# ksadov/FREUD

Measured on AMD Instinct MI355X. Metric: SAE train activations/sec (d=384 dict 8x), higher is better.
Workload: dtype bf16; 1 GPU; Whisper-tiny d=384 dict 8x (n=3072) L1 SAE train step, M=65536 rows/GPU/step, RAdam+cosine, x bfloat16 resident in HBM (BASELINE configs[1]); rows_per_gpu=65536, d_model=384, n_dict=3072, parallelism=dp1, dp=none

## Files before the change

freud_amd/csrc/engine.hip:

```cpp
#include <hip/hip_runtime.h>
#include <math.h>
#include <stdarg.h>
#include <stdio.h>
#include <string.h>

#include <algorithm>
#include <utility>
#include <vector>

#include "../../include/freud_sae.h"
#include "l1_kernels.h"
#include "gemm256.h"
#include "gemm256s.h"
#include "gemm256_fp8.h"
#include "l1_fp8.h"
#include "dp_kernels.h"
#include "p2p_exchange.h"
#include <rccl/rccl.h>
#include <mutex>
#include <unistd.h>

static thread_local bool g_force_gemm128 = false;
static thread_local bool g_no_stream = false;
static thread_local int g_device = 0;
// ... 49 lines not shown
  do {                                                                        \
    int rc_ = ensure_lds_attr(reinterpret_cast<const void*>(fn), (bytes), (device)); \
    if (rc_) return rc_;                                                      \
  } while (0)

static int grid_for(int64_t n, int cap, int per = 256) {
  const int64_t g = (n + per - 1) / per;
  return (int)(g < cap ? g : cap);
}

template <class F>
static int with_x_type(int x_dtype, const void* x, F&& f) {
  switch (x_dtype) {
    case SAE_DTYPE_F32: return f((const float*)x);
    case SAE_DTYPE_F16: return f((const _Float16*)x);
    case SAE_DTYPE_BF16: return f((const bf16_t*)x);
    default: return fail(SAE_ERR_INVALID, "unknown x_dtype %d", x_dtype);
  }
}

enum KernelId {
  KID_PREP_W = 0,
  KID_PREP_X,
  KID_ENC_FWD,
  KID_DEC_FWD,
  KID_FWD_FUSED,
  KID_DPRE,
  KID_DW,
  KID_BWD_FUSED,
  KID_REDUCE,
  KID_OPT,
  KID_TK_ENC,
  KID_TK_SELECT,
  KID_TK_DECODE,
  KID_TK_DDENSE,
  KID_TK_DWD,
  KID_TK_DWE,
  KID_TK_DSAE,
  KID_TK_AUX,
  KID_EXCHANGE,
  KID_STATS_XCHG,
  KID_STEP_TOTAL,
  KID_COACT_PACK,
  KID_COACT_UPDATE,
  KID_MANIP_SERIES,
  KID_MANIP_DECODE,
  KID_MANIP_APPLY,
  KID_LABEL_PACK,
  KID_LABEL_UPDATE,
  KID_COUNT
};
static const char* kKernelNames[KID_COUNT] = {"prep_w", "prep_x", "enc_fwd_gemm", "dec_fwd_gemm", "fwd_fused_gemm", "dpre_gemm",
                                              "dw_gemm", "bwd_fused_gemm", "reduce_grads", "clip_adam", "topk_enc_gemm", "topk_select",
                                              "topk_decode", "topk_ddense_gemm", "topk_dwdec_gemm", "topk_dwenc_gemm",
                                              "topk_dsaein_colsum", "topk_auxk_backward", "dp_exchange", "dp_stats_exchange",
                                              "fwd_bwd_total", "coact_pack", "coact_update", "manip_series", "manip_decode",
                                              "manip_apply", "label_pack", "label_update"};
constexpr int EV_RING = 64;

struct EvRing {
  hipEvent_t beg[EV_RING], end[EV_RING];
  int n = 0;
};

enum LastCall { LAST_FWD_BF16 = 0, LAST_FWD_E32, LAST_SEARCH, LAST_STATS, LAST_COACT, LAST_LABELS };

struct sae_ctx {
  sae_config cfg;
  int d, n, d_p, n_p;
  int64_t max_rows_p;
  int64_t nW;
  int64_t nparams;
  float *P = nullptr, *Mom = nullptr, *Var = nullptr;
  float* G = nullptr;
  bf16_t *Wb = nullptr, *Wt = nullptr;
  bool fp8 = false;
  bool fp8_bwd = false;
  unsigned char* dxh8 = nullptr;
  int row_pad = 128;
  unsigned char *x8 = nullptr, *c8 = nullptr, *W8 = nullptr, *W8t = nullptr;
  float *scal8 = nullptr, *x8_part = nullptr;
  bool use_fused_fwd = false;
  int fwd_variant = 2;
  bf16_t *xb = nullptr, *c = nullptr, *dxh = nullptr, *dpre = nullptr;
  bf16_t *dxhT = nullptr, *xT = nullptr;
  float *slab = nullptr, *db_part = nullptr, *l1_part = nullptr, *sq_part = nullptr, *scal = nullptr;
  double* gn_part = nullptr;
  float* cn_part = nullptr;
  bool cn_valid = false;
  bool wb_valid = false;
  float* cnorm = nullptr;
  bool wn_pending = false, wn_fwd_seen = false;
  sae_grad_ready_fn grad_ready = nullptr;
  void* grad_ready_user = nullptr;
  int dw_chunk_rows = 0;
  int dw_chunk_splits = 1;
  int dw_col_chunks = 1;
  int dw_col_splits = 1;
  float* cnt_part = nullptr;
  int gn_blocks = 0;
  bool step_fused_call = false;
  bool gn_valid = false;
  bool metrics_fresh = false;
  const bf16_t* xb_cur = nullptr;
  unsigned int* masked = nullptr;
  int dw_splits = 1;
  int dw_tail_tiles = 0, dw_tail_pieces = 0;
  float* dw_tail = nullptr;
  int bwd_splits = 1;
  int bwd_range_splits = 1;
  bool use_fused_bwd = false;
  bool topk = false;
  int k = 0, k_aux_cap = 0;
  int64_t rows_per_file = 0;
  double dead_threshold = 1e300;
  bf16_t *We_b = nullptr, *Wd_b = nullptr, *xs = nullptr, *pre = nullptr, *dense = nullptr, *aux_dense = nullptr;
  bf16_t *de_b = nullptr, *dh_b = nullptr;
  float *e = nullptr, *dh = nullptr, *e2_part = nullptr, *a2_part = nullptr, *dbd_part = nullptr, *ds_part = nullptr, *tkf = nullptr;
  int *top_idx = nullptr, *aux_idx = nullptr, *tk = nullptr;
  bf16_t *top_vals = nullptr, *aux_vals = nullptr, *multi_vals = nullptr;
  unsigned short* tile_max = nullptr;
  unsigned char* sel_flag = nullptr;
  bool dense_valid = false;
  bool multi_dense_valid = false;
  float* be_r = nullptr;
  int slab_splits = 1;
  bool aux_compact = false;
  int *tkd = nullptr, *dead_cols = nullptr, *vec_rank = nullptr;
  unsigned char* vec_bits = nullptr;
  bf16_t* Wdd_b = nullptr;
  float* aux_dbe_part = nullptr;
  int* dead_hint = nullptr;
  double* tv_part = nullptr;
  long long* nfsf = nullptr;
  long long* dbe_fx = nullptr;
  bool topk_sparse_da = false;
  bool topk_csc = false;
  unsigned short* csc_counts = nullptr;
  unsigned int *csc_block_off = nullptr, *csc_total = nullptr, *csc_start = nullptr, *csc_item_start = nullptr, *csc_item_latent = nullptr;
  unsigned int* csc_multi = nullptr;
  CscEntry* csc_entries = nullptr;
  float *csc_part = nullptr, *csc_pbe = nullptr;
  int64_t csc_max_items = 0;
  bool multi = false;
  int k4 = 0;
  bf16_t *multi_dense = nullptr, *dm_b = nullptr;
  int* multi_idx = nullptr;
  float *em = nullptr, *m2_part = nullptr;
  unsigned char* dead = nullptr;
  double* stats = nullptr;
  int64_t stats_cap = 0, stats_n = 0;
  unsigned int* stats_part = nullptr;
  int dp_world = 0;
  bool dist = false;
  ncclComm_t comm = nullptr;
  hipStream_t comm_stream = nullptr;
  hipEvent_t ev_x = nullptr, ev_stats = nullptr, ev_done = nullptr;
  hipEvent_t ev_range[16] = {};
  int ev_range_i = 0;
  int payload = SAE_DTYPE_F32;
  bf16_t* Gb = nullptr;
  bool grads_in_bf16 = false;
  int dist_error = 0;
  char dist_errmsg[256] = "";
  bool p2p = false;
  int p2p_rank = 0;
// ... 296 lines not shown
        if (r.beg[i]) (void)hipEventDestroy(r.beg[i]);
        if (r.end[i]) (void)hipEventDestroy(r.end[i]);
      }
  delete c;
}

extern "C" int sae_create(const sae_config* cfg, sae_ctx** out) {
  if (!cfg || !out) return fail(SAE_ERR_INVALID, "null argument");
  *out = nullptr;
  if (cfg->variant != SAE_VARIANT_L1 && cfg->variant != SAE_VARIANT_TOPK)
    return fail(SAE_ERR_INVALID, "Invalid autoencoder variant: %d, must be 'l1' or 'topk'", cfg->variant);
  if (cfg->variant == SAE_VARIANT_TOPK && (cfg->k <= 0 || cfg->k > cfg->n_dict || cfg->k > 1024))
    return fail(SAE_ERR_INVALID, "topk: k=%d must be in [1, min(n_dict, 1024)]", cfg->k);
  if (cfg->variant == SAE_VARIANT_TOPK && cfg->multi_topk && (4 * cfg->k > cfg->n_dict || 4 * cfg->k > 1024))
    return fail(SAE_ERR_INVALID, "topk: multi_topk selects 4k = %d latents, must be <= min(n_dict, 1024)", 4 * cfg->k);
  if (cfg->variant != SAE_VARIANT_TOPK && cfg->multi_topk)
    return fail(SAE_ERR_INVALID, "multi_topk is a TopK option");
  if (cfg->variant == SAE_VARIANT_TOPK && cfg->d_model > 1536)
    return fail(SAE_ERR_INVALID, "topk: d_model=%d above the 1536 the sparse decoder is built for", cfg->d_model);
  if (cfg->d_model <= 0 || cfg->n_dict <= 0 || cfg->max_rows <= 0)
    return fail(SAE_ERR_INVALID, "d_model, n_dict and max_rows must be positive");
  if (cfg->optimizer != SAE_OPT_RADAM && cfg->optimizer != SAE_OPT_ADAM)
    return fail(SAE_ERR_INVALID, "Invalid optimizer: %d, must be 'radam' or 'adam'", cfg->optimizer);
  int ndev = 0;
  HIP_TRY(hipGetDeviceCount(&ndev));
  if (cfg->device_id < 0 || cfg->device_id >= ndev) return fail(SAE_ERR_INVALID, "device_id %d out of range", cfg->device_id);
  HIP_TRY(hipSetDevice(cfg->device_id));
  g_device = cfg->device_id;

  if (cfg->precision != SAE_PREC_BF16 && cfg->precision != SAE_PREC_FP8 && cfg->precision != SAE_PREC_FP8_BWD)
    return fail(SAE_ERR_INVALID, "Invalid precision: %d, must be SAE_PREC_BF16, SAE_PREC_FP8 or SAE_PREC_FP8_BWD", cfg->precision);
  if (cfg->precision != SAE_PREC_BF16 && cfg->variant != SAE_VARIANT_L1)
    return fail(SAE_ERR_INVALID, "fp8 encoder / decoder GEMMs exist for the L1 variant only");

  sae_ctx* c = new sae_ctx();
  c->cfg = *cfg;
  c->d = cfg->d_model;
  c->n = cfg->n_dict;
  c->fp8 = cfg->precision != SAE_PREC_BF16;
  c->fp8_bwd = cfg->precision == SAE_PREC_FP8_BWD;
  const int pad = c->fp8 ? 256 : 128;
  c->row_pad = pad;
  c->d_p = (int)round_up(c->d, pad);
  c->n_p = (int)round_up(c->n, pad);
  c->max_rows_p = round_up(cfg->max_rows, pad);
  c->nW = (int64_t)c->d_p * c->n_p;
  c->nparams = c->nW + c->n_p;
  c->topk = cfg->variant == SAE_VARIANT_TOPK;
  if (const char* fg = getenv("FREUD_P2P_FINEGRAINED")) c->finegrained = atoi(fg) == 1;
  const int64_t Mp = c->max_rows_p;
  if (c->topk) {
    int rc_tk = topk_create(c, Mp);
    if (rc_tk) {
      sae_destroy(c);
      return rc_tk;
    }
    *out = c;
    return SAE_OK;
  }
  g_force_gemm128 = cfg->force_gemm128 == 1;
  c->no_stream = g_no_stream = cfg->debug_flags == 86 || (getenv("FREUD_GEMM_STREAM") && atoi(getenv("FREUD_GEMM_STREAM")) == 0);
  c->dw_splits = choose_splits(c->d_p / 128, c->n_p / 128, 2 * Mp / 64);
  if (const char* ov = getenv("FREUD_DW_SPLITS")) {
    const int v = atoi(ov);
    if (v >= 1 && v <= 64) c->dw_splits = v;
  }
  c->dw_chunk_rows = c->d_p >= 1024 ? 512 : c->d_p;
  if (!g_force_gemm128 && c->d_p % 256 == 0 && c->n_p % 256 == 0 && (c->d_p / 256) * (c->n_p / 256) >= 256 && !getenv("FREUD_DW_SPLITS") &&
      c->cfg.debug_flags != 81) {
    gemm_tail_plan((c->d_p / 256) * (c->n_p / 256), (int)(2 * Mp / 64), c->dw_tail_tiles, c->dw_tail_pieces);
    if ((c->d_p / 256) * (c->n_p / 256) % 256 == 0) c->dw_tail_tiles = c->dw_tail_pieces = -1;
  }
  c->dw_chunk_splits = choose_splits(c->dw_chunk_rows / 128, c->n_p / 128, 2 * Mp / 64);
  if (c->d_p >= 1024 && c->n_p % 256 == 0)
    for (int q = 4; q >= 2; --q)
      if ((c->n_p / 256) % q == 0) {
        c->dw_col_chunks = q;
        break;
      }
  c->dw_col_splits = choose_splits(c->d_p / 128, c->n_p / 128 / c->dw_col_chunks, 2 * Mp / 64);
  c->use_fused_bwd = (c->d_p == BF_D) && cfg->force_generic != 1 && !c->fp8;
  c->use_fused_fwd = (c->d_p == FF_D) && cfg->force_generic != 1 && !c->fp8;
  if (const char* fv = getenv("FREUD_FWD")) c->fwd_variant = atoi(fv) == 1 ? 1 : 2;
  c->bwd_splits = fused_bwd_splits(c->n_p / BF_BN, (int)(Mp / BF_BM), c->n_p);
  c->bwd_range_splits = c->bwd_splits;
  for (int r = 2; r <= 4; ++r)
    if ((c->n_p / BF_BN) % r == 0) {
      const int sp = fused_bwd_splits(c->n_p / BF_BN / r, (int)(Mp / BF_BM), c->n_p / r);
      if (sp > c->bwd_range_splits) c->bwd_range_splits = sp;
    }
  int slab_splits = c->use_fused_bwd ? (c->bwd_range_splits > c->dw_splits ? c->bwd_range_splits : c->dw_splits) : c->dw_splits;
  if (c->use_fused_bwd && c->cfg.debug_flags != 83 && !getenv("FREUD_BWD_UNIFORM")) {
    const int ntiles = c->n_p / BF_BN, cus = 256;
    const int m = (32 * ntiles + cus - 1) / cus, grid = (32 * ntiles + m - 1) / m;
    int pmax = 1;
    for (int j = 0; j < ntiles; ++j) pmax = bal_pieces(j, m) > pmax ? bal_pieces(j, m) : pmax;
    const int steps = (int)(Mp / BF_BM), q = (steps + 31) / 32;
    const double slab_steps = (double)c->n_p * BF_D * 8.0 / 4.0e12 / 1.43e-6;
    const double cost_bal = (double)m * q + 5.0 + (32 % m ? 3.5 : 0.0) + (32.0 / m + (32 % m ? 1.0 : 0.0)) * slab_steps;
    const int sp = c->bwd_splits, rounds = (ntiles * sp + 255) / 256;
    const double cost_uni = rounds * ((double)((steps + sp - 1) / sp) + 5.0) + sp * slab_steps;
    if (cost_bal < cost_uni * 0.995 && pmax <= 64 && grid <= 4096) {
      c->bal_m = m;
      c->bal_grid = grid;
      if (pmax > slab_splits) slab_splits = pmax;
      std::vector<int> order(grid);
      for (int k = 0; k < grid; ++k) order[k] = k;
      std::stable_sort(order.begin(), order.end(), [m](int a_, int b_) { return (a_ * m) % 32 < (b_ * m) % 32; });
      std::vector<short> map(grid);
      int pos = 0;
      for (int x = 0; x < 8; ++x) {
        const int len = grid / 8 + (x < grid % 8 ? 1 : 0);
        for (int i = 0; i < len; ++i) map[8 * i + x] = (short)order[pos++];
      }
      hipError_t e_ = hipMalloc((void**)&c->bal_map, (size_t)grid * 2);
      if (e_ == hipSuccess) e_ = hipMemcpy(c->bal_map, map.data(), (size_t)grid * 2, hipMemcpyHostToDevice);
      if (e_ != hipSuccess) {
        int rc_ = fail(SAE_ERR_HIP, "balanced backward: workgroup table: %s", hipGetErrorString(e_));
        sae_destroy(c);
        return rc_;
      }
    }
  }
  {
    const int64_t need = (int64_t)(c->dw_chunk_splits > c->dw_col_splits ? c->dw_chunk_splits : c->dw_col_splits);
    if (need > slab_splits) slab_splits = (int)need;
  }
  const int64_t db_rows = (Mp / 128) > 64 ? (Mp / 128) : 64;

#define ALLOC(ptr, bytes)                                   \
  do {                                                      \
    hipError_t e_ = hipMalloc((void**)&(ptr), (bytes));     \
    if (e_ != hipSuccess) {                                 \
      int rc_ = fail(SAE_ERR_HIP, "hipMalloc(%lld bytes) for %s failed: %s", (long long)(bytes), #ptr, \
                     hipGetErrorString(e_));                \
      sae_destroy(c);                                       \
      return rc_;                                           \
    }                                                       \
  } while (0)
  ALLOC(c->P, c->nparams * 4);
  ALLOC(c->Mom, c->nparams * 4);
  ALLOC(c->Var, c->nparams * 4);
  if (c->finegrained) {
    hipError_t e_ = peer_visible_malloc(c, (void**)&c->G, (size_t)(c->nparams + SAE_NUM_METRICS) * 4);
    if (e_ == hipSuccess) e_ = peer_visible_malloc(c, (void**)&c->stats, (size_t)DP_STATS_HEAD * 8);
    if (e_ != hipSuccess) {
      int rc_ = fail(SAE_ERR_HIP, "fine-grained allocation of the gradient / statistics buffers failed: %s", hipGetErrorString(e_));
      sae_destroy(c);
      return rc_;
    }
  } else {
    ALLOC(c->G, (c->nparams + SAE_NUM_METRICS) * 4);
  }
  ALLOC(c->Wb, c->nW * 2);
  ALLOC(c->Wt, c->nW * 2);
  ALLOC(c->xb, Mp * c->d_p * 2);
  ALLOC(c->c, Mp * c->n_p * 2 + 4096);
  ALLOC(c->dxh, Mp * c->d_p * 2);
  ALLOC(c->dpre, Mp * c->n_p * 2);
  if (!c->use_fused_bwd && !g_force_gemm128 && c->d_p % 256 == 0 && c->n_p % 256 == 0 && Mp % 64 == 0 &&
      getenv("FREUD_DW_ROWA") && atoi(getenv("FREUD_DW_ROWA")) == 1) {
    ALLOC(c->dxhT, Mp * c->d_p * 2);
    ALLOC(c->xT, Mp * c->d_p * 2);
  }
  ALLOC(c->slab, (int64_t)slab_splits * c->nW * 4);
  ALLOC(c->db_part, db_rows * c->n_p * 4);
// ... 829 lines not shown
  const int d = c->d, d_p = c->d_p;
  const int grid = grid_for(Mp * (d_p / 8), 2048);
  if (d % 8 == 0 && (reinterpret_cast<uintptr_t>(x) & 15) == 0)
    hipLaunchKernelGGL((prep_x_kernel<T, true>), dim3(grid), dim3(256), 0, s, x, c->xb, c->masked, M, d, Mp, d_p);
  else
    hipLaunchKernelGGL((prep_x_kernel<T, false>), dim3(grid), dim3(256), 0, s, x, c->xb, c->masked, M, d, Mp, d_p);
  return grid;
}

static GemmArgs enc_gemm_args(const sae_ctx* c, const bf16_t* xb, int64_t Mp) {
  GemmArgs g{};
  g.A0 = xb; g.B0 = c->Wt; g.lda = c->d_p; g.ldb = c->d_p;
  g.nbm = (int)(Mp / 128); g.nbn = c->n_p / 128; g.ktiles0 = g.ktiles = c->d_p / 64; g.splits = 1;
  return g;
}

template <typename T>
static auto launch_encoder(sae_ctx* c, const GemmArgs& g, int64_t M, hipStream_t s) {
  EpiEnc e{};
  e.c = c->c; e.bias = c->P + c->nW; e.l1_part = c->l1_part; e.M = M; e.n_p = c->n_p; e.nbn = g.nbn;
  if (gemm_streams<OP_ROW, OP_ROW, EpiEnc>(g)) HIP_TRY(hipMemsetAsync(c->l1_part, 0, (size_t)g.nbm * g.nbn * 4, s));
  ev_begin(c, KID_ENC_FWD, s);
  const int rc = launch_gemm<OP_ROW, OP_ROW>(g, e, s);
  ev_end(c, KID_ENC_FWD, s);
  return rc;
}

template <typename T> static constexpr bool x_dtype_is_bf16() { return false; }
template <> constexpr bool x_dtype_is_bf16<bf16_t>() { return true; }

template <typename T>
static int forward_impl(sae_ctx* c, const T* x, int64_t M, int64_t Mp, hipStream_t s, bool need_backward) {
  const int d = c->d, d_p = c->d_p, n_p = c->n_p;
  const float alpha = (float)c->cfg.recon_alpha;
  float* W = c->P;
  float* b = c->P + c->nW;

  ev_begin(c, KID_PREP_W, s);
  prep_weights_l1(c, s);
  if (c->fp8) hipLaunchKernelGGL(fp8_cast_w_kernel, dim3(n_p / 64, d_p / 64), dim3(256), 0, s, W, c->W8, c->W8t, d_p, n_p);
  ev_end(c, KID_PREP_W, s);

  ev_begin(c, KID_PREP_X, s);
  const bool alias_x = c->use_fused_fwd && sizeof(T) == 2 && x_dtype_is_bf16<T>() && d == d_p && M == Mp &&
                       (reinterpret_cast<uintptr_t>(x) & 15) == 0;
  c->xb_cur = alias_x ? reinterpret_cast<const bf16_t*>(x) : c->xb;
  if (!alias_x) {
    const int grid = launch_prep_x(c, x, M, Mp, s);
    if (!c->use_fused_fwd) {
      const double* gs = (need_backward && c->dp_world > 0) ? c->stats : nullptr;
      if (gs && c->dist) HIP_TRY(hipStreamWaitEvent(s, c->ev_stats, 0));
      hipLaunchKernelGGL(finalize_count_kernel, dim3(1), dim3(256), 0, s, c->masked, grid, c->scal, M, d, alpha, gs);
    }
  }
  if (c->fp8) {
    const int sgrid = (int)((Mp / 4) < 1024 ? (Mp / 4) : 1024);
    hipLaunchKernelGGL(fp8_x_stats_kernel, dim3(sgrid), dim3(256), 0, s, c->xb, Mp, d_p, c->x8_part);
    hipLaunchKernelGGL(fp8_scales_kernel, dim3(1), dim3(256), 0, s, c->x8_part, sgrid, b, c->n, c->scal8);
    const int64_t n8 = Mp * (d_p / 8);
    hipLaunchKernelGGL(fp8_quant_x_kernel, dim3(grid_for(n8, 2048)), dim3(256), 0, s, c->xb, c->x8, n8, c->scal8);
  }
  ev_end(c, KID_PREP_X, s);

  int rc;
  if (c->use_fused_fwd) {
    const int lds = FF_LDS_BYTES;
    FwdFusedArgs a{};
    a.xb = c->xb_cur; a.x = x; a.Wt = c->Wt; a.bias = b; a.cnt_part = c->cnt_part; a.c = c->c; a.dxh = c->dxh;
    a.l1_part = c->l1_part; a.sq_part = c->sq_part; a.M = M; a.d = d; a.n_p = n_p; a.ntiles = n_p / FF_BN;
    a.c_rows = c->max_rows_p;
    const int full_wgs = (int)(M / FF_BM), all_wgs = (int)(Mp / FF_BM);
    auto launch = [&](auto kern, int blocks, int block_offset) -> int {
      LDS_ATTR(kern, 160 * 1024, g_device);
      a.block_offset = block_offset;
      hipLaunchKernelGGL(kern, dim3(blocks), dim3(256), lds, s, a);
      return SAE_OK;
    };
    ev_begin(c, KID_FWD_FUSED, s);
    int rcl = SAE_OK;
    if (full_wgs > 0 && c->cfg.debug_flags == 65 && c->fwd_variant == 1) {
      a.stamps = reinterpret_cast<unsigned long long*>(c->dpre);
      rcl = launch(fwd_fused_d384_kernel<T, false, true>, full_wgs, 0);
    } else if (c->fwd_variant == 2) {
      if (full_wgs > 0 && c->cfg.debug_flags == 65) {
        a.stamps = reinterpret_cast<unsigned long long*>(c->dpre);
        rcl = launch(fwd_fused2_d384_kernel<T, false, true>, full_wgs, 0);
      } else if (full_wgs > 0) rcl = launch(fwd_fused2_d384_kernel<T, false>, full_wgs, 0);
      if (!rcl && all_wgs > full_wgs) rcl = launch(fwd_fused2_d384_kernel<T, true>, all_wgs - full_wgs, full_wgs);
      if (rcl) return rcl;
      ev_end(c, KID_FWD_FUSED, s);
      HIP_TRY(hipGetLastError());
      return SAE_OK;
    } else if (full_wgs > 0) {
      rcl = launch(fwd_fused_d384_kernel<T, false, false>, full_wgs, 0);
    }
    if (!rcl && all_wgs > full_wgs) rcl = launch(fwd_fused_d384_kernel<T, true, false>, all_wgs - full_wgs, full_wgs);
    if (rcl) return rcl;
    ev_end(c, KID_FWD_FUSED, s);
    HIP_TRY(hipGetLastError());
    return SAE_OK;
  }
  if (c->fp8) {
    {
      Gemm8Args g{};
      g.A = c->x8; g.B = c->W8t; g.lda = d_p; g.ldb = d_p;
      g.nbm = (int)(Mp / 256); g.nbn = n_p / 256; g.ktiles = d_p / 128;
      EpiEnc8 e{};
      e.c = c->c; e.c8 = c->c8; e.bias = b; e.scal8 = c->scal8; e.l1_part = c->l1_part; e.M = M; e.n_p = n_p; e.nbn = n_p / 128;
      if (gemm8_streams<EpiEnc8>(g)) HIP_TRY(hipMemsetAsync(c->l1_part, 0, (size_t)(Mp / 128) * (n_p / 128) * 4, s));
      ev_begin(c, KID_ENC_FWD, s);
      rc = launch_gemm8(g, e, s);
      ev_end(c, KID_ENC_FWD, s);
      if (rc) return rc;
    }
    {
      Gemm8Args g{};
      g.A = c->c8; g.B = c->W8; g.lda = n_p; g.ldb = n_p;
      g.nbm = (int)(Mp / 256); g.nbn = d_p / 256; g.ktiles = n_p / 128;
      EpiDec<T> e{};
      e.x = x; e.dxh = c->dxh; e.scal = c->scal; e.sq_part = c->sq_part; e.M = M; e.d = d; e.d_p = d_p; e.nbn = d_p / 128;
      e.vec_all = (M == Mp && d == d_p && d % 4 == 0 && (reinterpret_cast<uintptr_t>(x) % (4 * sizeof(T))) == 0) ? 1 : 0;
      e.vscale = c->scal8 + S8_INV_DEC;
      ev_begin(c, KID_DEC_FWD, s);
      rc = launch_gemm8(g, e, s);
      ev_end(c, KID_DEC_FWD, s);
      if (rc) return rc;
    }
    if (need_backward && c->dxhT) {
      hipLaunchKernelGGL(transpose_bf16_kernel, dim3((unsigned)(Mp / 64), d_p / 64), dim3(256), 0, s, c->dxh, c->dxhT, Mp, d_p);
      hipLaunchKernelGGL(transpose_bf16_kernel, dim3((unsigned)(Mp / 64), d_p / 64), dim3(256), 0, s, c->xb_cur, c->xT, Mp, d_p);
      HIP_TRY(hipGetLastError());
    }
    return SAE_OK;
  }
  rc = launch_encoder<T>(c, enc_gemm_args(c, c->xb_cur, Mp), M, s);
  if (rc) return rc;
  {
    GemmArgs g{};
    g.A0 = c->c; g.B0 = c->Wb; g.lda = n_p; g.ldb = n_p;
    g.nbm = (int)(Mp / 128); g.nbn = d_p / 128; g.ktiles0 = g.ktiles = n_p / 64; g.splits = 1;
    g.group_m = 4;
    EpiDec<T> e{};
    e.x = x; e.dxh = c->dxh; e.scal = c->scal; e.sq_part = c->sq_part; e.M = M; e.d = d; e.d_p = d_p; e.nbn = g.nbn;
    e.vec_all = (M == Mp && d == d_p && d % 4 == 0 && (reinterpret_cast<uintptr_t>(x) % (4 * sizeof(T))) == 0) ? 1 : 0;
    ev_begin(c, KID_DEC_FWD, s);
    rc = launch_gemm<OP_ROW, OP_ROW>(g, e, s);
    ev_end(c, KID_DEC_FWD, s);
    if (rc) return rc;
  }
  if (need_backward && c->dxhT) {
    hipLaunchKernelGGL(transpose_bf16_kernel, dim3((unsigned)(Mp / 64), d_p / 64), dim3(256), 0, s, c->dxh, c->dxhT, Mp, d_p);
    hipLaunchKernelGGL(transpose_bf16_kernel, dim3((unsigned)(Mp / 64), d_p / 64), dim3(256), 0, s, c->xb_cur, c->xT, Mp, d_p);
    HIP_TRY(hipGetLastError());
  }
  return SAE_OK;
}

template <typename T>
static int fwd_bwd_impl(sae_ctx* c, const T* x, int64_t M, hipStream_t s, bool backward) {
  const int d = c->d, d_p = c->d_p, n_p = c->n_p;
  const int64_t Mp = round_up(M, c->row_pad);
  const float alpha = (float)c->cfg.recon_alpha;
  const double* gs = (backward && c->dp_world > 0) ? c->stats : nullptr;
  ev_begin(c, KID_STEP_TOTAL, s);
  int rc = forward_impl<T>(c, x, M, Mp, s, backward);
  if (rc) return rc;
  const bool fold_finalize = c->use_fused_fwd && c->use_fused_bwd && backward && gs == nullptr && c->bwd_ranges == 1 &&
                             c->cfg.debug_flags != 78;
  if (c->use_fused_fwd && !fold_finalize) {
    StatsPush push{};
// ... 1724 lines not shown
```

freud_amd/csrc/fwd_fused.h:

```cpp
#pragma once
#include <type_traits>
constexpr int FF_DMA_G0 = 15;
constexpr int FF_DMA_G1 = 19;
constexpr int FF_DMA_G2 = 23;

#include "bwd_fused.h"

constexpr int FF_D = 384;
constexpr int FF_BM = 128;
constexpr int FF_BN = 32;
constexpr int FF_WT_BYTES = FF_BN * FF_D * 2;
constexpr int FF_DEPTH = 4;
constexpr int FF_RING_BYTES = FF_DEPTH * FF_WT_BYTES;
constexpr int FF_CST_BYTES = 4 * 2 * 4096;
constexpr int FF_FIXED_LDS = FF_RING_BYTES + FF_CST_BYTES;
constexpr int FF_BIAS_RING_TILES = 8;
constexpr int FF_BIAS_RING_BYTES = FF_BIAS_RING_TILES * FF_BN * 4;
constexpr int FF_LDS_BYTES = FF_FIXED_LDS + FF_BIAS_RING_BYTES;

struct FwdFusedArgs {
  const bf16_t* xb;
  const void* x;
  const bf16_t* Wt;
  const float* bias;
  float* cnt_part;
  bf16_t* c;
  bf16_t* dxh;
  float* l1_part;
  float* sq_part;
  int64_t M;
  int d, n_p, ntiles;
  int block_offset;
  unsigned long long* stamps;
  int64_t c_rows;
};

template <typename T, bool PAD, bool STAMP = false>
__global__ __launch_bounds__(256, 1) void fwd_fused_d384_kernel(FwdFusedArgs a) {
  extern __shared__ __attribute__((aligned(16))) char smem[];
  const int t = threadIdx.x, lane = t & 63, w = t >> 6;
  const int arow = lane & 31, ah = lane >> 5;
  const int wg = blockIdx.x + a.block_offset;
  const int64_t m0 = (int64_t)wg * FF_BM + 32 * w;
  const int64_t mrow = m0 + arow;
  const bool row_ok = mrow < a.M;
  char* cst = smem + FF_RING_BYTES + w * 8192;
  float* bias_s = reinterpret_cast<float*>(smem + FF_FIXED_LDS);
  unsigned long long clk_k0 = 0;
  if (STAMP) clk_k0 = __builtin_amdgcn_s_memtime();

  bf16x8 xfrag[24];
  {
    const bf16_t* xp = a.xb + mrow * FF_D + 8 * ah;
#pragma unroll
    for (int kk = 0; kk < 24; ++kk) xfrag[kk] = *reinterpret_cast<const bf16x8*>(xp + 16 * kk);
  }
  if (t < 2 * FF_BN) bias_s[t] = a.bias[t];
  for (int i = t; i < FF_WT_BYTES / 16; i += 256)
    reinterpret_cast<u32x4*>(smem + 3 * FF_WT_BYTES)[i] = u32x4{0u, 0u, 0u, 0u};

  f32x16 acc[12];
#pragma unroll
  for (int i = 0; i < 12; ++i)
#pragma unroll
    for (int r = 0; r < 16; ++r) acc[i][r] = 0.f;

  unsigned voff_t[6], loff_t[6];
#pragma unroll
  for (int i = 0; i < 6; ++i) {
    const int inst = w + 4 * i, sub = inst >> 3, row = 4 * (inst & 7) + (lane >> 4), pc = lane & 15;
    const int ch = pc ^ (((row & 3) << 2) | ((row >> 2) & 3));
    voff_t[i] = (unsigned)(row * (FF_D * 2) + (sub * 16 + ch) * 16);
    loff_t[i] = (unsigned)__builtin_amdgcn_readfirstlane(sub * 8192 + (inst & 7) * 1024);
  }
  typedef __attribute__((address_space(3))) char* lptr_t;
  const unsigned smem_base = (unsigned)(uintptr_t)(lptr_t)smem;
  auto dma_pair = [&](int p, int jt, int st) {
    const bf16_t* src = a.Wt + (int64_t)jt * FF_BN * FF_D;
    const unsigned dst = smem_base + st * FF_WT_BYTES;
    glds16_x2(src, src, voff_t[2 * p], voff_t[2 * p + 1], (unsigned)__builtin_amdgcn_readfirstlane((int)(dst + loff_t[2 * p])),
              (unsigned)__builtin_amdgcn_readfirstlane((int)(dst + loff_t[2 * p + 1])));
  };
  const int last = a.ntiles - 1;
#pragma unroll
  for (int q = 0; q < 2; ++q)
#pragma unroll
    for (int p = 0; p < 3; ++p) dma_pair(p, q <= last ? q : last, q);
#pragma unroll
  for (int kk = 0; kk < 24; ++kk) asm volatile("" : "+v"(xfrag[kk]));
  asm volatile("s_waitcnt vmcnt(0)" ::: "memory");
  __syncthreads();

  int roff[8], toff[8];
#pragma unroll
  for (int i = 0; i < 8; ++i) roff[i] = dual_off(arow, 2 * i + ah);
  {
    const int g = (lane >> 4) & 1, q = (lane & 15) >> 2, p = lane & 3;
#pragma unroll
    for (int i = 0; i < 8; ++i) {
      const int col = 32 * (i >> 1) + 16 * g + 4 * p;
      const int r = 4 * ah + q + 8 * (i & 1);
      toff[i] = dual_off(r, col >> 3) + (col & 7) * 2;
    }
  }
  typedef __attribute__((ext_vector_type(8))) short s16x8;
  auto tr_pair = [&](const char* p0, const char* p1) -> bf16x8 {
    const s16x4 lo = __builtin_amdgcn_ds_read_tr16_b64_v4i16(LDS_PTR(s16x4, p0));
    const s16x4 hi = __builtin_amdgcn_ds_read_tr16_b64_v4i16(LDS_PTR(s16x4, p1));
    const s16x8 v = __builtin_shufflevector(lo, hi, 0, 1, 2, 3, 4, 5, 6, 7);
    return __builtin_bit_cast(bf16x8, v);
  };
  const int drow_l = lane >> 3, dch = lane & 7;
  bf16_t* cdrain = a.c + (m0 + drow_l) * a.n_p + dch * 8;

  float l1_acc = 0.f;
// ... 269 lines not shown
```

freud_amd/csrc/fwd_fused2.h:

```cpp
#pragma once
#include "fwd_fused.h"

typedef __attribute__((ext_vector_type(2))) float f32x2_t;

template <typename T, bool PAD, bool STAMP = false>
__global__ __launch_bounds__(256, 1) void fwd_fused2_d384_kernel(FwdFusedArgs a) {
  extern __shared__ __attribute__((aligned(16))) char smem[];
  const int t = threadIdx.x, lane = t & 63, w = t >> 6;
  const int arow = lane & 31, ah = lane >> 5;
  const int wg = blockIdx.x + a.block_offset;
  const int64_t m0 = (int64_t)wg * FF_BM + 32 * w;
  const int64_t mrow = m0 + arow;
  const bool row_ok = mrow < a.M;
  char* cst = smem + FF_RING_BYTES;
  float* bias_s = reinterpret_cast<float*>(smem + FF_FIXED_LDS);
  unsigned long long clk_k0 = 0, clk_t0 = 0, clk_r0 = 0, clk_t1 = 0;
  if (STAMP) clk_k0 = __builtin_amdgcn_s_memtime();

  typedef __attribute__((ext_vector_type(2))) unsigned short us2_t;
  constexpr unsigned MASK_BITS2 = std::is_same<T, bf16_t>::value ? 0xBF80BF80u : 0xBC00BC00u;
  constexpr bool SCAN_EARLY = !PAD && std::is_same<T, bf16_t>::value;
  bool wany_early = false;

  bf16x8 xfrag[24];
  unsigned voff_t[6], loff_t[6];
#pragma unroll
  for (int i = 0; i < 6; ++i) {
    const int inst = w + 4 * i, sub = inst >> 3, row = 4 * (inst & 7) + (lane >> 4), pc = lane & 15;
    const int ch = pc ^ (((row & 3) << 2) | ((row >> 2) & 3));
    voff_t[i] = (unsigned)(row * (FF_D * 2) + (sub * 16 + ch) * 16);
    loff_t[i] = (unsigned)__builtin_amdgcn_readfirstlane(sub * 8192 + (inst & 7) * 1024);
  }
  typedef __attribute__((address_space(3))) char* lptr_t;
  const unsigned smem_base = (unsigned)(uintptr_t)(lptr_t)smem;
  auto dma_pair = [&](int p, int jt, int st) {
    const bf16_t* src = a.Wt + (int64_t)jt * FF_BN * FF_D;
    const unsigned dst = smem_base + st * FF_WT_BYTES;
    glds16_x2(src, src, voff_t[2 * p], voff_t[2 * p + 1], (unsigned)__builtin_amdgcn_readfirstlane((int)(dst + loff_t[2 * p])),
              (unsigned)__builtin_amdgcn_readfirstlane((int)(dst + loff_t[2 * p + 1])));
  };
  auto dma_one = [&](int k, int jt, int st) {
    const bf16_t* src = a.Wt + (int64_t)jt * FF_BN * FF_D;
    glds16(src, voff_t[k], (unsigned)__builtin_amdgcn_readfirstlane((int)(smem_base + st * FF_WT_BYTES + loff_t[k])));
  };
  const int last = a.ntiles - 1;
#pragma unroll
  for (int q = 0; q < 3; ++q)
#pragma unroll
    for (int p = 0; p < 3; ++p) dma_pair(p, q <= last ? q : last, q);
  static_assert(2 * FF_BN == 64, "one 4-byte piece per lane of wave 0");
  if (w == 0) glds4(a.bias, (unsigned)(lane * 4), (unsigned)__builtin_amdgcn_readfirstlane((int)(smem_base + FF_FIXED_LDS)));
  {
    const bf16_t* xp = a.xb + mrow * FF_D + 8 * ah;
#pragma unroll
    for (int kk = 0; kk < 24; ++kk) xfrag[kk] = *reinterpret_cast<const bf16x8*>(xp + 16 * kk);
  }
  for (int i = t; i < FF_WT_BYTES / 16; i += 256) reinterpret_cast<u32x4*>(smem + 3 * FF_WT_BYTES)[i] = u32x4{0u, 0u, 0u, 0u};
  for (int i = t; i < FF_CST_BYTES / 16; i += 256) reinterpret_cast<u32x4*>(cst)[i] = u32x4{0u, 0u, 0u, 0u};

  f32x16 acc[12];
#pragma unroll
  for (int i = 0; i < 12; ++i)
#pragma unroll
    for (int r = 0; r < 16; ++r) acc[i][r] = 0.f;

  if (SCAN_EARLY) {
    us2_t mz = {0xFFFFu, 0xFFFFu};
#pragma unroll
    for (int kk = 0; kk < 24; ++kk) {
      const u32x4 xw = __builtin_bit_cast(u32x4, xfrag[kk]);
#pragma unroll
      for (int c = 0; c < 4; ++c) mz = __builtin_elementwise_min(mz, __builtin_bit_cast(us2_t, xw[c] ^ MASK_BITS2));
    }
    wany_early = __builtin_amdgcn_ballot_w64((mz[0] == 0) | (mz[1] == 0)) != 0ull;
  }
#pragma unroll
  for (int kk = 0; kk < 24; ++kk) asm volatile("" : "+v"(xfrag[kk]));
  asm volatile("s_waitcnt vmcnt(0)" ::: "memory");
  __syncthreads();

  int roff[8];
#pragma unroll
  for (int i = 0; i < 8; ++i) roff[i] = dual_off(arow, 2 * i + ah);
  int aoff0[6], aoff1[6];
  {
    const int g = (lane >> 4) & 1, q = (lane & 15) >> 2, p = lane & 3;
#pragma unroll
    for (int f = 0; f < 6; ++f) {
      const int ks = f / 3, dt = 3 * w + f % 3;
      const int col = 32 * (dt & 3) + 16 * g + 4 * p;
      const int r0 = 4 * ah + q, r1 = r0 + 8;
      const int base = (dt >> 2) * 8192 + ks * 4096;
      aoff0[f] = base + dual_off(r0, col >> 3) + (col & 7) * 2;
      aoff1[f] = base + dual_off(r1, col >> 3) + (col & 7) * 2;
    }
  }
  typedef __attribute__((ext_vector_type(8))) short s16x8;
  auto tr_pair = [&](const char* p0, const char* p1) -> bf16x8 {
    const s16x4 lo = __builtin_amdgcn_ds_read_tr16_b64_v4i16(LDS_PTR(s16x4, p0));
    const s16x4 hi = __builtin_amdgcn_ds_read_tr16_b64_v4i16(LDS_PTR(s16x4, p1));
    const s16x8 v = __builtin_shufflevector(lo, hi, 0, 1, 2, 3, 4, 5, 6, 7);
    return __builtin_bit_cast(bf16x8, v);
  };
  auto swz = [](int row) { return (row & 7) ^ ((row >> 1) & 1) ^ ((row >> 4) & 1); };
  int boff[4];
#pragma unroll
  for (int i = 0; i < 4; ++i) boff[i] = arow * 128 + (((4 * (i >> 1) + 2 * (i & 1) + ah) ^ swz(arow)) << 4);
  const int wrow = w * 4096;
  const int drow_l = lane >> 3, dch = lane & 7;
  int doff0, doff1;
  {
    const int tl = dch >> 2, s = (dch & 3) >> 1, u = dch & 1;
    doff0 = drow_l * 128 + (((4 * tl + 2 * s + 0) ^ swz(drow_l)) << 4) + 8 * u;
    doff1 = drow_l * 128 + (((4 * tl + 2 * s + 1) ^ swz(drow_l)) << 4) + 8 * u;
  }
  auto dpiece = [](int off, int p) { return (p & 2) ? (off ^ 16) : off; };
  bf16_t* cdrain = a.c + (m0 + drow_l) * a.n_p + dch * 8;

  float l1_acc = 0.f;

  f32x16 Sn;
#pragma unroll
  for (int r = 0; r < 16; ++r) Sn[r] = 0.f;
#pragma unroll
  for (int kk = 0; kk < 24; ++kk) {
    const bf16x8 fa = *reinterpret_cast<const bf16x8*>(smem + (kk >> 3) * 8192 + roff[kk & 7]);
    Sn = __builtin_amdgcn_mfma_f32_32x32x16_bf16(fa, xfrag[kk], Sn, 0, 0, 0);
  }

  constexpr int RING = 8;
  const char *rlo[8], *rhi[8];
#pragma unroll
  for (int i = 0; i < 8; ++i) {
    rlo[i] = smem + roff[i];
    rhi[i] = smem + 2 * FF_WT_BYTES + roff[i];
// ... 156 lines not shown
      o[0] = o[1] = o[2] = 0; o[3] = (unsigned long long)a.ntiles; o[4] = t1 - clk_t0; o[5] = r1 - clk_r0; o[6] = clk_t0 - clk_k0;
    }
  }
  Bq[2] = dec_b(1, 1, 2);
#pragma unroll
  for (int m = 0; m < 24; ++m) {
    if (m == 3 || m == 4 || m == 5) Afr[m] = dec_a(3, m);
    if (m % 3 == 0 && m / 3 + 3 <= 7) Bq[(m / 3 + 3) & 3] = dec_b(1, 1, m / 3 + 3);
    __builtin_amdgcn_sched_barrier(0);
    const int ks = m / 12, mb = (m % 12) / 3, dtl = m % 3;
    acc[4 * dtl + mb] = __builtin_amdgcn_mfma_f32_32x32x16_bf16(Afr[3 * ks + dtl], Bq[(4 * ks + mb) & 3], acc[4 * dtl + mb], 0, 0, 0);
    __builtin_amdgcn_sched_barrier(0);
  }
  {
    const char* cst_r = cst + (((a.ntiles >> 1) - 1) & 1) * 16384 + wrow;
#pragma unroll
    for (int p = 0; p < 4; ++p) {
      const uint2 lo = *reinterpret_cast<const uint2*>(cst_r + p * 1024 + dpiece(doff0, p));
      const uint2 hi = *reinterpret_cast<const uint2*>(cst_r + p * 1024 + dpiece(doff1, p));
      __builtin_nontemporal_store(u32x4{lo.x, lo.y, hi.x, hi.y},
                                  reinterpret_cast<u32x4*>(cdrain + (int64_t)(8 * p) * a.n_p + 64 * ((a.ntiles >> 1) - 1)));
    }
  }
  __builtin_amdgcn_sched_barrier(0);
  asm volatile("s_waitcnt vmcnt(4) lgkmcnt(0)" ::: "memory");
  __builtin_amdgcn_s_barrier();
  __builtin_amdgcn_sched_barrier(0);

  unsigned long long clk_e0 = 0, clk_e1 = 0, clk_e2 = 0;
  if (STAMP) clk_e0 = __builtin_amdgcn_s_memtime();
  float sq = 0.f, plain = 0.f, nmask = 0.f;
  float msq = 0.f;
  f32x2_t plain2 = {0.f, 0.f};
  typedef __attribute__((ext_vector_type(4))) T Tx4;
  const bool vec_ok = (a.d == FF_D) && ((reinterpret_cast<uintptr_t>(a.x) & (sizeof(T) * 4 - 1)) == 0);
  constexpr int FF_DXH_PITCH = FF_D * 2 + 16;
  static_assert(128 * FF_DXH_PITCH <= FF_FIXED_LDS, "the dx_hat staging must fit the idle LDS");
  char* stg = smem;
  constexpr bool X_VIA_LDS = !PAD && sizeof(T) == 2;
  constexpr bool X_FROM_FRAGS = X_VIA_LDS && std::is_same<T, bf16_t>::value;
  unsigned* mflag = reinterpret_cast<unsigned*>(smem + FF_FIXED_LDS + 64);
  bool blk_masked = true;
  if (X_FROM_FRAGS && vec_ok && reinterpret_cast<const void*>(a.x) == reinterpret_cast<const void*>(a.xb)) {
    char* srow_w = stg + (32 * w + arow) * FF_DXH_PITCH + 16 * ah;
    us2_t mz = {0xFFFFu, 0xFFFFu};
#pragma unroll
    for (int kk = 0; kk < 24; ++kk) {
      *reinterpret_cast<bf16x8*>(srow_w + 32 * kk) = xfrag[kk];
      if (!SCAN_EARLY) {
        const u32x4 xw = __builtin_bit_cast(u32x4, xfrag[kk]);
#pragma unroll
        for (int c = 0; c < 4; ++c) mz = __builtin_elementwise_min(mz, __builtin_bit_cast(us2_t, xw[c] ^ MASK_BITS2));
      }
    }
    const bool wany = SCAN_EARLY ? wany_early : __builtin_amdgcn_ballot_w64((mz[0] == 0) | (mz[1] == 0)) != 0ull;
    if (lane == 0) mflag[w] = wany ? 1u : 0u;
    __syncthreads();
    const u32x4 f = *reinterpret_cast<const u32x4*>(mflag);
    blk_masked = (f[0] | f[1] | f[2] | f[3]) != 0u;
  } else
  if (X_VIA_LDS && vec_ok) {
    const char* xblk = reinterpret_cast<const char*>(reinterpret_cast<const T*>(a.x) + m0 * FF_D);
    us2_t mz = {0xFFFFu, 0xFFFFu};
#pragma unroll
    for (int p0 = 0; p0 < 24; p0 += 4) {
      u32x4 xr[4];
#pragma unroll
      for (int pc = 0; pc < 4; ++pc) xr[pc] = *reinterpret_cast<const u32x4*>(xblk + (p0 + pc) * 1024 + lane * 16);
#pragma unroll
      for (int pc = 0; pc < 4; ++pc) {
        const int off = (p0 + pc) * 1024 + lane * 16, r = off / (FF_D * 2), cb = off - r * (FF_D * 2);
        *reinterpret_cast<u32x4*>(stg + (32 * w + r) * FF_DXH_PITCH + cb) = xr[pc];
#pragma unroll
        for (int c = 0; c < 4; ++c) mz = __builtin_elementwise_min(mz, __builtin_bit_cast(us2_t, xr[pc][c] ^ MASK_BITS2));
      }
    }
    const bool wany = __builtin_amdgcn_ballot_w64((mz[0] == 0) | (mz[1] == 0)) != 0ull;
    if (lane == 0) mflag[w] = wany ? 1u : 0u;
    __syncthreads();
    const u32x4 f = *reinterpret_cast<const u32x4*>(mflag);
    blk_masked = (f[0] | f[1] | f[2] | f[3]) != 0u;
  }
  if (STAMP) clk_e1 = __builtin_amdgcn_s_memtime();
  auto residual = [&](auto notest_tag) {
  constexpr bool NOTEST = decltype(notest_tag)::value;
  constexpr bool FENCE = NOTEST && X_VIA_LDS;
  constexpr bool PIPE = FENCE && std::is_same<T, bf16_t>::value;
  Tx4 xq[2][4];
  auto xload = [&](int g, Tx4 (&dst)[4]) {
    const char* sr = stg + (32 * (g / 3) + arow) * FF_DXH_PITCH + (96 * w + 32 * (g % 3) + 4 * ah) * 2;
#pragma unroll
    for (int k = 0; k < 4; ++k) dst[k] = *reinterpret_cast<const Tx4*>(sr + 16 * k);
  };
  if constexpr (PIPE) xload(0, xq[0]);
#pragma unroll
  for (int mb = 0; mb < 4; ++mb) {
    const int64_t grow = (int64_t)wg * FF_BM + 32 * mb + arow;
    const bool ok = !PAD || grow < a.M;
    const float rmask = ok ? 1.f : 0.f;
    const T* xrow = reinterpret_cast<const T*>(a.x) + (ok ? grow : a.M - 1) * a.d;
    char* srow = stg + (32 * mb + arow) * FF_DXH_PITCH;
#pragma unroll
    for (int dtl = 0; dtl < 3; ++dtl) {
      const int dbase = 96 * w + 32 * dtl + 4 * ah;
      if (NOTEST || vec_ok) {
        const int g = 3 * mb + dtl;
        if constexpr (FENCE) {
          if (g > 0) __builtin_amdgcn_sched_barrier(0);
          if (PIPE && g + 1 < 12) xload(g + 1, xq[(g + 1) & 1]);
        }
        Tx4 xv[4];
#pragma unroll
        for (int k = 0; k < 4; ++k)
          xv[k] = PIPE ? xq[g & 1][k]
                       : (X_VIA_LDS ? *reinterpret_cast<const Tx4*>(srow + (dbase + 8 * k) * 2) : *reinterpret_cast<const Tx4*>(xrow + dbase + 8 * k));
        if (!PAD) {
          if constexpr (NOTEST && X_VIA_LDS) {
            if constexpr (std::is_same<T, bf16_t>::value) {
              uint2 ow[4];
#pragma unroll
              for (int k = 0; k < 4; ++k) {
                const uint2 xw = __builtin_bit_cast(uint2, xv[k]);
#pragma unroll
                for (int pp = 0; pp < 2; ++pp) {
                  const unsigned xd = pp ? xw.y : xw.x;
                  const unsigned rb = __builtin_bit_cast(unsigned, __builtin_convertvector(
                      f32x2_t{acc[4 * dtl + mb][4 * k + 2 * pp], acc[4 * dtl + mb][4 * k + 2 * pp + 1]}, bf16x2));
                  const f32x2_t rf = {__uint_as_float(rb << 16), __uint_as_float(rb & 0xFFFF0000u)};
                  const f32x2_t xf = {__uint_as_float(xd << 16), __uint_as_float(xd & 0xFFFF0000u)};
                  f32x2_t e2, d2;
                  asm("v_pk_add_f32 %0, %1, %2 neg_lo:[0,1] neg_hi:[0,1]" : "=v"(e2) : "v"(rf), "v"(xf));
                  asm("v_pk_fma_f32 %0, %1, %1, %0" : "+v"(plain2) : "v"(e2));
                  asm("v_pk_add_f32 %0, %1, %1" : "=v"(d2) : "v"(e2));
                  const unsigned ob = __builtin_bit_cast(unsigned, __builtin_convertvector(d2, bf16x2));
                  if (pp) ow[k].y = ob; else ow[k].x = ob;
                }
              }
#pragma unroll
              for (int k = 0; k < 4; ++k) *reinterpret_cast<uint2*>(srow + (dbase + 8 * k) * 2) = ow[k];
              continue;
            }
            bf16x4 o[4];
#pragma unroll
            for (int k = 0; k < 4; ++k)
#pragma unroll
              for (int q = 0; q < 4; ++q) {
                const float xf = (float)xv[k][q];
                const float e = bf16_round(acc[4 * dtl + mb][4 * k + q]) - xf;
                plain = __builtin_fmaf(e, e, plain);
                o[k][q] = (bf16_t)(e + e);
              }
#pragma unroll
            for (int k = 0; k < 4; ++k) *reinterpret_cast<bf16x4*>(srow + (dbase + 8 * k) * 2) = o[k];
            continue;
          }
          bf16x4 o[4];
          unsigned nm_i = 0u;
#pragma unroll
          for (int k = 0; k < 4; ++k)
#pragma unroll
            for (int q = 0; q < 4; ++q) {
              const float xf = (float)xv[k][q];
              const float e = bf16_round(acc[4 * dtl + mb][4 * k + q]) - xf;
              const bool mk = xf == -1.0f;
              const float em = mk ? e : 0.0f, ek = mk ? 0.0f : e;
              plain = __builtin_fmaf(e, e, plain);
// ... 3 lines not shown
            }
          nmask += (float)nm_i;
#pragma unroll
          for (int k = 0; k < 4; ++k) *reinterpret_cast<bf16x4*>(srow + (dbase + 8 * k) * 2) = o[k];
          continue;
        }
#pragma unroll
        for (int k = 0; k < 4; ++k) {
          bf16x4 o;
#pragma unroll
          for (int q = 0; q < 4; ++q) {
            const float xf = (float)xv[k][q];
            const float e = bf16_round(acc[4 * dtl + mb][4 * k + q]) - xf;
            const float e2 = e * e;
            plain += rmask * e2;
            const float keep = (xf != -1.0f) ? rmask : 0.f;
            nmask += rmask - keep;
            sq += keep * e2;
            o[q] = (bf16_t)(keep * (e * 2.0f));
          }
          *reinterpret_cast<bf16x4*>(srow + (dbase + 8 * k) * 2) = o;
        }
      } else {
#pragma unroll
        for (int k = 0; k < 4; ++k) {
          bf16x4 o;
#pragma unroll
          for (int q = 0; q < 4; ++q) {
            const int dd = dbase + 8 * k + q;
            const bool valid = dd < a.d;
            const float xf = (float)xrow[valid ? dd : a.d - 1];
            const float e = bf16_round(acc[4 * dtl + mb][4 * k + q]) - xf;
            const float e2 = valid ? e * e : 0.f;
            plain += rmask * e2;
            const float keep = (valid && xf != -1.0f) ? rmask : 0.f;
            nmask += (valid ? rmask : 0.f) - keep;
            sq += keep * e2;
            o[q] = (bf16_t)(keep * (e * 2.0f));
          }
          *reinterpret_cast<bf16x4*>(srow + (dbase + 8 * k) * 2) = o;
        }
      }
    }
  }
  };
  if (X_VIA_LDS && vec_ok && !blk_masked) residual(std::true_type{}); else residual(std::false_type{});
  if (STAMP) clk_e2 = __builtin_amdgcn_s_memtime();
  __syncthreads();
  {
    char* gblk = reinterpret_cast<char*>(a.dxh + m0 * FF_D);
#pragma unroll
    for (int pc = 0; pc < 24; ++pc) {
      const int off = pc * 1024 + lane * 16, r = off / (FF_D * 2), cb = off - r * (FF_D * 2);
      *reinterpret_cast<u32x4*>(gblk + off) = *reinterpret_cast<const u32x4*>(stg + (32 * w + r) * FF_DXH_PITCH + cb);
    }
  }
  plain += plain2[0] + plain2[1];
  if (!PAD && vec_ok) sq = plain - msq;
  float* red = reinterpret_cast<float*>(smem + FF_FIXED_LDS);
  {
    const float v0 = wave_sum(l1_acc), v1 = wave_sum(sq), v2 = wave_sum(plain), v3 = wave_sum(nmask);
    if (lane == 0) *reinterpret_cast<f32x4*>(red + 4 * w) = f32x4{v0, v1, v2, v3};
  }
  lds_barrier();
  const float l1s = ((red[0] + red[4]) + red[8]) + red[12];
  const float sqs = ((red[1] + red[5]) + red[9]) + red[13];
  const float pls = ((red[2] + red[6]) + red[10]) + red[14];
  const float nms = ((red[3] + red[7]) + red[11]) + red[15];
  if (STAMP && lane == 0) {
    unsigned long long* o = a.stamps + ((int64_t)wg * 4 + w) * 8;
    const unsigned long long te = __builtin_amdgcn_s_memtime();
    o[7] = te - clk_k0;
    o[0] = clk_e0 - clk_t1; o[1] = clk_e1 - clk_e0; o[2] = clk_e2 - clk_e1;
#ifdef FF2_WAITSTAMP
    o[0] = ws_vm; o[1] = ws_bar; o[2] = ws_gap;
#endif
  }
  if (t == 0) {
    a.cnt_part[wg] = nms;
    a.l1_part[wg] = l1s;
    a.sq_part[2 * wg] = sqs;
    a.sq_part[2 * wg + 1] = pls;
  }
}
```

Measured before the change: 120.5 million activations/s.

## Make fused forward kernel persistent with cross-tile prefetch of next x rows

The fused d=384 forward kernel becomes persistent. It launches one workgroup per CU (or a grid size set by an environment variable) and loops over row tiles with a grid stride. During the residual phase of the current tile it loads the next tile's x fragments into registers, which hides the x load latency and removes the per-workgroup launch and ramp-up cost. In exchange, register pressure rises, workgroups may become serialized when tail work is unbalanced, and the loop must stay correct across iterations, including LDS reuse after the lgkmcnt wait.

```diff
diff --git a/freud_amd/csrc/engine.hip b/freud_amd/csrc/engine.hip
--- a/freud_amd/csrc/engine.hip
+++ b/freud_amd/csrc/engine.hip
@@ -155,6 +155,8 @@
   float *scal8 = nullptr, *x8_part = nullptr;
   bool use_fused_fwd = false;
   int fwd_variant = 2;
+  int num_cus = 0;
+  int fwd_grid = 0;
   bf16_t *xb = nullptr, *c = nullptr, *dxh = nullptr, *dpre = nullptr;
   bf16_t *dxhT = nullptr, *xT = nullptr;
   float *slab = nullptr, *db_part = nullptr, *l1_part = nullptr, *sq_part = nullptr, *scal = nullptr;
@@ -617,6 +619,11 @@
   c->use_fused_bwd = (c->d_p == BF_D) && cfg->force_generic != 1 && !c->fp8;
   c->use_fused_fwd = (c->d_p == FF_D) && cfg->force_generic != 1 && !c->fp8;
   if (const char* fv = getenv("FREUD_FWD")) c->fwd_variant = atoi(fv) == 1 ? 1 : 2;
+  if (hipDeviceGetAttribute(&c->num_cus, hipDeviceAttributeMultiprocessorCount, cfg->device_id) != hipSuccess || c->num_cus <= 0) {
+    sae_destroy(c);
+    return fail(SAE_ERR_INVALID, "device %d does not report its number of compute units", cfg->device_id);
+  }
+  if (const char* fg = getenv("FREUD_FWD_GRID")) c->fwd_grid = atoi(fg) > 0 ? atoi(fg) : 0;
   c->bwd_splits = fused_bwd_splits(c->n_p / BF_BN, (int)(Mp / BF_BM), c->n_p);
   c->bwd_range_splits = c->bwd_splits;
   for (int r = 2; r <= 4; ++r)
@@ -1612,10 +1619,13 @@
       a.stamps = reinterpret_cast<unsigned long long*>(c->dpre);
       rcl = launch(fwd_fused_d384_kernel<T, false, true>, full_wgs, 0);
     } else if (c->fwd_variant == 2) {
+      const int want = c->fwd_grid > 0 ? c->fwd_grid : c->num_cus;
+      const int G = full_wgs < want ? full_wgs : want;
+      a.wg_end = full_wgs;
       if (full_wgs > 0 && c->cfg.debug_flags == 65) {
         a.stamps = reinterpret_cast<unsigned long long*>(c->dpre);
-        rcl = launch(fwd_fused2_d384_kernel<T, false, true>, full_wgs, 0);
-      } else if (full_wgs > 0) rcl = launch(fwd_fused2_d384_kernel<T, false>, full_wgs, 0);
+        rcl = launch(fwd_fused2_d384_kernel<T, false, true>, G, 0);
+      } else if (full_wgs > 0) rcl = launch(fwd_fused2_d384_kernel<T, false>, G, 0);
       if (!rcl && all_wgs > full_wgs) rcl = launch(fwd_fused2_d384_kernel<T, true>, all_wgs - full_wgs, full_wgs);
       if (rcl) return rcl;
       ev_end(c, KID_FWD_FUSED, s);
diff --git a/freud_amd/csrc/fwd_fused.h b/freud_amd/csrc/fwd_fused.h
--- a/freud_amd/csrc/fwd_fused.h
+++ b/freud_amd/csrc/fwd_fused.h
@@ -31,6 +31,7 @@
   int64_t M;
   int d, n_p, ntiles;
   int block_offset;
+  int wg_end;
   unsigned long long* stamps;
   int64_t c_rows;
 };
diff --git a/freud_amd/csrc/fwd_fused2.h b/freud_amd/csrc/fwd_fused2.h
--- a/freud_amd/csrc/fwd_fused2.h
+++ b/freud_amd/csrc/fwd_fused2.h
@@ -6,12 +6,6 @@
 template <typename T, bool PAD, bool STAMP = false>
 __global__ __launch_bounds__(256, 1) void fwd_fused2_d384_kernel(FwdFusedArgs a) {
   extern __shared__ __attribute__((aligned(16))) char smem[];
-  const int t = threadIdx.x, lane = t & 63, w = t >> 6;
-  const int arow = lane & 31, ah = lane >> 5;
-  const int wg = blockIdx.x + a.block_offset;
-  const int64_t m0 = (int64_t)wg * FF_BM + 32 * w;
-  const int64_t mrow = m0 + arow;
-  const bool row_ok = mrow < a.M;
   char* cst = smem + FF_RING_BYTES;
   float* bias_s = reinterpret_cast<float*>(smem + FF_FIXED_LDS);
   unsigned long long clk_k0 = 0, clk_t0 = 0, clk_r0 = 0, clk_t1 = 0;
@@ -20,9 +14,17 @@
   typedef __attribute__((ext_vector_type(2))) unsigned short us2_t;
   constexpr unsigned MASK_BITS2 = std::is_same<T, bf16_t>::value ? 0xBF80BF80u : 0xBC00BC00u;
   constexpr bool SCAN_EARLY = !PAD && std::is_same<T, bf16_t>::value;
-  bool wany_early = false;
+  constexpr bool EARLY_X = !PAD && std::is_same<T, bf16_t>::value;
 
   bf16x8 xfrag[24];
+  int wg = blockIdx.x + a.block_offset;
+  bool x_early = false;
+#pragma unroll 1
+  for (;;) {
+  int t = threadIdx.x;
+  asm volatile("" : "+v"(t));
+  const int lane = t & 63, w = t >> 6;
+  const int arow = lane & 31, ah = lane >> 5;
   unsigned voff_t[6], loff_t[6];
 #pragma unroll
   for (int i = 0; i < 6; ++i) {
@@ -44,13 +46,17 @@
     glds16(src, voff_t[k], (unsigned)__builtin_amdgcn_readfirstlane((int)(smem_base + st * FF_WT_BYTES + loff_t[k])));
   };
   const int last = a.ntiles - 1;
+  const int64_t m0 = (int64_t)wg * FF_BM + 32 * w;
+  const int64_t mrow = m0 + arow;
+  const bool row_ok = mrow < a.M;
+  bool wany_early = false;
 #pragma unroll
   for (int q = 0; q < 3; ++q)
 #pragma unroll
     for (int p = 0; p < 3; ++p) dma_pair(p, q <= last ? q : last, q);
   static_assert(2 * FF_BN == 64, "one 4-byte piece per lane of wave 0");
   if (w == 0) glds4(a.bias, (unsigned)(lane * 4), (unsigned)__builtin_amdgcn_readfirstlane((int)(smem_base + FF_FIXED_LDS)));
-  {
+  if (!x_early) {
     const bf16_t* xp = a.xb + mrow * FF_D + 8 * ah;
 #pragma unroll
     for (int kk = 0; kk < 24; ++kk) xfrag[kk] = *reinterpret_cast<const bf16x8*>(xp + 16 * kk);
@@ -373,6 +379,15 @@
     blk_masked = (f[0] | f[1] | f[2] | f[3]) != 0u;
   }
   if (STAMP) clk_e1 = __builtin_amdgcn_s_memtime();
+  const int wg_next = wg + (int)gridDim.x;
+  const bool more = !PAD && wg_next < a.wg_end;
+  if (EARLY_X && more) {
+    __builtin_amdgcn_sched_barrier(0);
+    const bf16_t* xp = a.xb + ((int64_t)wg_next * FF_BM + 32 * w + arow) * FF_D + 8 * ah;
+#pragma unroll
+    for (int kk = 0; kk < 24; ++kk) xfrag[kk] = *reinterpret_cast<const bf16x8*>(xp + 16 * kk);
+    __builtin_amdgcn_sched_barrier(0);
+  }
   auto residual = [&](auto notest_tag) {
   constexpr bool NOTEST = decltype(notest_tag)::value;
   constexpr bool FENCE = NOTEST && X_VIA_LDS;
@@ -542,4 +557,10 @@
     a.sq_part[2 * wg] = sqs;
     a.sq_part[2 * wg + 1] = pls;
   }
+  if (PAD || !more) break;
+  asm volatile("s_waitcnt lgkmcnt(0)" ::: "memory");
+  wg = wg_next;
+  x_early = EARLY_X;
+  if (STAMP) clk_k0 = __builtin_amdgcn_s_memtime();
+  }
 }
```

After: 120.7 million activations/s (median of 6 runs). No clear change (+0.2%).
